# prannaykaul/lvc

Measured on AMD Instinct MI355X. Metric: img/s COCO 800x1333 R50-FPN inference (GeneralizedRCNN.forward(batched_inputs) -> Instances, 1000 proposals, 100 detections), higher is better.
Workload: dtype f32 (conv/GEMM inner products on the fp16 / bf16 matrix cores through fp32-accurate operand splits: two-way fp16 with main + cross fp32 accumulators for the 3x3 and wide 1x1 / FC layers, three-way bf16 for the rest; final boxes/scores closer to the fp64 evaluation than the reference's fp32 CPU path,; 1 GPU; COCO-detection R50-FPN inference, bs=8 synthetic 3x800x1333 per GPU, 1000 pre/post-NMS proposals per level/image, 80 classes, conditioned random-init weights; batch_per_gpu=8, global_batch=8, parallelism=dp1

## Files before the change

include/lvc_amd.h:

```cpp
#ifndef LVC_AMD_H
#define LVC_AMD_H

#ifdef __cplusplus
extern "C" {
#endif

#define LVC_OK 0
#define LVC_ERR_INVALID 1
#define LVC_ERR_HIP 2

int lvc_abi_version(void);
const char* lvc_last_error(void);
void lvc_set_error(const char* fmt, ...);

long long lvc_conv_workspace_bytes(void);
long long lvc_conv_range_words_offset(void);
void lvc_set_range_slot(int slot);
int lvc_range_slot(void);
int lvc_range_slots(void);
int lvc_conv2d_nhwc_f32(const float* x, const float* w_packed, const float* scale, const float* shift,
                        const float* residual, float* y, int N, int H, int W, int C, int K, int R, int S,
                        int stride, int pad, int Kg, int relu, int res_mode, int ldy, int ldr, int mode,
                        void* workspace, void* stream);

int lvc_conv2d_nhwc_bf16x3(const float* x, const unsigned short* w_split, const float* scale, const float* shift,
                           const float* residual, float* y, int N, int H, int W, int C, int K, int R, int S,
                           int stride, int pad, int Kg, int relu, int res_mode, int ldy, int ldr, void* workspace,
                           void* stream);

int lvc_conv3x3_nhwc_bf16x3(const float* x, const unsigned short* w_split, const float* scale, const float* shift,
                            const float* residual, float* y, int N, int H, int W, int C, int K, int Kg, int relu,
                            int res_mode, int ldy, int ldr, void* workspace, void* stream);

int lvc_conv3x3_nhwc_f16x2(const float* x, const unsigned short* w_split, const float* scale, const float* shift,
                           const float* residual, float* y, int N, int H, int W, int C, int K, int Kg, int relu,
                           int res_mode, int ldy, int ldr, void* workspace, void* stream);
int lvc_conv3x3_nhwc_f16s1(const float* x, const unsigned short* w_split, const float* scale, const float* shift,
                           const float* residual, float* y, int N, int H, int W, int C, int K, int Kg, int relu,
                           int res_mode, int ldy, int ldr, void* workspace, void* stream);
int lvc_conv3x3_nhwc_f16x2_pipe(const float* x, const unsigned short* w_split, const float* scale, const float* shift,
                                const float* residual, float* y, int N, int H, int W, int C, int K, int Kg, int relu,
                                int res_mode, int ldy, int ldr, void* workspace, void* stream);
int lvc_conv3x3_nhwc_f16_levels(int oneacc, const float* const* xs, float* const* ys, const int* Hs, const int* Ws, int L,
                                const unsigned short* w_split, const float* scale, const float* shift, int N, int C, int K, int Kg,
                                int relu, void* workspace, void* stream);
int lvc_conv3x3_nhwc_f16_levels_pred(int oneacc, const float* const* xs, float* const* ys, const int* Hs, const int* Ws, int L,
                                     const unsigned short* w_split, const float* scale, const float* shift, int N, int C, int K, int Kg,
                                     int relu, const unsigned short* pred_w, const float* pred_scale, const float* pred_shift, int pred_K,
                                     int pred_rows, int pred_ld, int pred_slot, void* workspace, void* stream);
int lvc_conv3x3_nhwc_f16_layers(int oneacc, const float* const* xs, float* const* ys, const int* Hs, const int* Ws, int L,
                                const unsigned short* const* ws, const float* const* scales, const float* const* shifts, int N, int C,
                                int K, int Kg, int relu, void* workspace, void* stream);
void lvc_set_wino_streamk(int mode);
void lvc_set_nms_reduce_global(int on);
void lvc_set_select_onelaunch(int mode);
int lvc_select_onelaunch(void);
void lvc_set_halo_test_hooks(int ph, int pw, int force);
int lvc_conv3x3_nhwc_wino(const float* x, const unsigned short* u, const float* scale, const float* shift, float* y, int N, int H, int W,
                          int C, int K, int Kpad, int relu, int ldy, void* workspace, void* stream);
int lvc_conv3x3_nhwc_wino_pred(const float* x, const unsigned short* u, const float* scale, const float* shift, float* y, int N, int H,
                               int W, int C, int K, int Kpad, int relu, int ldy, const unsigned short* pred_w, const float* pred_scale,
                               const float* pred_shift, int pred_K, int pred_rows, int pred_slot, void* workspace, void* stream);
int lvc_conv1x1_nhwc_f16x2_pipe(const float* x, const unsigned short* w_split, const float* scale, const float* shift,
                                const float* residual, float* y, int N, int H, int W, int C, int K, int stride, int relu,
                                int res_mode, int ldy, int ldr, void* workspace, void* stream);
int lvc_conv1x1_nhwc_f16s1(const float* x, const unsigned short* w_split, const float* scale, const float* shift,
                           const float* residual, float* y, int N, int H, int W, int C, int K, int stride, int relu,
                           int res_mode, int ldy, int ldr, void* workspace, void* stream);
int lvc_conv3x3_nhwc_f16s1_presplit(const float* x, const unsigned short* w_split, const float* scale, const float* shift, void* y,
                                    int N, int H, int W, int C, int K, int Kg, int next_slot, void* workspace, void* stream);
int lvc_conv1x1_nhwc_f16s1_presplit(const void* x, const unsigned short* w_split, const float* scale, const float* shift,
                                    const float* residual, float* y, int N, int H, int W, int C, int K, int relu,
                                    int res_mode, int ldy, int ldr, void* workspace, void* stream);
int lvc_conv1x1_nhwc_f16s1_w2(const float* x, const unsigned short* w_split, const float* scale, const float* shift,
                              const float* residual, float* y, int N, int H, int W, int C, int K, int Kpad, int stride, int relu,
                              int res_mode, int ldy, int ldr, void* workspace, void* stream);
int lvc_conv1x1_chain_nhwc_f16s1(const float* x, int ldx, const unsigned short* wa, int wa_rows, const float* sa, const float* ta,
                                 const float* residual, int ldr, float* y1, int ldy1, int relu1, const unsigned short* wb,
                                 int wb_rows, const float* sb, const float* tb, float* y2, int ldy2, int relu2, int M, int K1,
                                 int N1, int N2, void* workspace, void* stream);
int lvc_bottleneck_nhwc_f16s1(const float* x, int ldx, float* y, int ldy, int N, int H, int W, int cin, int proj,
                              const unsigned short* w, const float* s1, const float* t1, const float* s2, const float* t2,
                              const float* s3, const float* t3, void* workspace, void* stream);
int lvc_split_weights_rowscaled(const float* wp, int rows, int Kg, void* planes_out, float* row_factor, void* stream);

int lvc_conv2d_nhwc_f16x2(const float* x, const unsigned short* w_split, const float* scale, const float* shift,
                          const float* residual, float* y, int N, int H, int W, int C, int K, int R, int S,
                          int stride, int pad, int Kg, int relu, int res_mode, int ldy, int ldr, void* workspace,
                          void* stream);
int lvc_conv2d_nhwc_f16x2_dma(const float* x, const unsigned short* w_split, const float* scale, const float* shift,
                          const float* residual, float* y, int N, int H, int W, int C, int K, int R, int S,
                          int stride, int pad, int Kg, int relu, int res_mode, int ldy, int ldr, void* workspace,
                          void* stream);

int lvc_stem_conv_pool_nhwc4_f16x2(const float* x, const unsigned short* w_split, const float* scale, const float* shift,
                                   float* y, int N, int H, int W, int Kpad, int relu, int* d_error_word,
                                   float* y2 , int ldy2, void* stream);

int lvc_preprocess_nhwc4(const void* image, int dtype, int h, int w, const float* mean3, const float* std3,
                         float* out, int Hp, int Wp, void* stream);
int lvc_preprocess_batch_nhwc4(const void* const* images, int dtype, const int* hs, const int* ws, int B, const float* mean3,
                               const float* std3, float* out, int Hp, int Wp, void* stream);

int lvc_resize_bilinear_u8(const unsigned char* image, int H, int W, int new_h, int new_w, const int* xb, const int* xk,
                           int kxs, const int* yb, const int* yk, int kys, unsigned char* tmp, unsigned char* out_u8,
                           float* out_nhwc4, int Hp, int Wp, const float* mean3, const float* std3, void* stream);
int lvc_tta_resize_u8(const unsigned char* image, int H, int W, long long sy, long long sx, long long sc, const long long* hjobs,
                      int n_h, const long long* vjobs, int n_v, const float* mean3, const float* std3, void* stream);
long long lvc_tta_merge_workspace_bytes(int B, int Nmax);
int lvc_tta_merge(const float* boxes, const float* scores, const int* classes, const int* counts, int topk_in, const float* params,
                  const int* tab, int B, int Nmax, float score_thresh, double nms_thresh, int topk_out, float* ob, float* osc, int* ocl,
                  int* ocount, void* workspace, long long workspace_bytes, void* stream);
// ... 203 lines not shown
```

lvc_amd/_lib.py:

```python
import ctypes
import os

_HERE = os.path.dirname(os.path.abspath(__file__))
_SO = os.environ.get("LVC_AMD_LIB") or os.path.join(_HERE, "liblvc_amd.so")
_lib = None

c_void_p = ctypes.c_void_p
c_int = ctypes.c_int
c_float = ctypes.c_float
c_double = ctypes.c_double
c_longlong = ctypes.c_longlong


class LvcNativeError(RuntimeError):
    pass


def lib():
    global _lib
    if _lib is None:
        if not os.path.exists(_SO):
            raise ImportError(
                "lvc_amd: native library {} not found; build it with "
                "`python -c 'import __graft_entry__ as g; g.build()'` or `make -C lvc_amd/csrc` "
                "(there is no CPU fallback)".format(_SO)
            )
        L = ctypes.CDLL(_SO)
        L.lvc_last_error.restype = ctypes.c_char_p
        L.lvc_batched_nms_workspace_bytes.restype = c_longlong
        L.lvc_tta_merge_workspace_bytes.restype = c_longlong
        L.lvc_group_norm_workspace_bytes.restype = c_longlong
        L.lvc_abi_version.restype = c_int
        L.lvc_set_wino_streamk.restype = None
        if os.environ.get("LVC_WINO_STREAMK", "0") != "0":
            L.lvc_set_wino_streamk(c_int(int(os.environ["LVC_WINO_STREAMK"])))
        L.lvc_set_nms_reduce_global.restype = None
        L.lvc_set_halo_test_hooks.restype = None
        if os.environ.get("LVC_NMS_REDUCE_GLOBAL", "0") != "0":
            L.lvc_set_nms_reduce_global(c_int(1))
        L.lvc_set_select_onelaunch.restype = None
        if os.environ.get("LVC_SELECT_ONELAUNCH", "3") != "3":
            L.lvc_set_select_onelaunch(c_int(int(os.environ["LVC_SELECT_ONELAUNCH"])))
        _lib = L
    return _lib


def check(status, what=""):
    if status != 0:
        msg = lib().lvc_last_error().decode("utf-8", "replace")
        lib().lvc_set_range_slot(0)
        raise LvcNativeError("{} failed (status {}): {}".format(what or "lvc_amd native call", status, msg))


def ptr(t):
    if t is None:
        return c_void_p(0)
    return c_void_p(t.data_ptr())


def current_stream(device=None):
    import torch

    return c_void_p(torch.cuda.current_stream(device).cuda_stream)
```

lvc_amd/csrc/conv3x3_wino.hip:

```cpp
#include "conv_common.h"
#include <stdlib.h>
#include <type_traits>

#define WN_NT 512
#define WN_PAIRS 128
#define WN_CH 128
#define WN_VROWS 160
#define WN_PP (WN_VROWS * 32)
#define WN_VBUF (8 * WN_PP)
#define WN_USLOT (8 * WN_CH * 32)
#define WN_SMEM (2 * WN_VBUF + 2 * WN_USLOT)

struct WinoArgs {
  const float* x;
  const unsigned short* u;
  const float* scale;
  const float* shift;
  float* y;
  int* flags;
  float* partials;
  int N, H, W, C, K, Kpad, ldy, relu;
  int PH, PWP, lg_pwp, tiles_x, tiles_y, tiles_n, ntiles, nk, err_index;
  int units_per_worker, nworkers;
  unsigned x_bytes, y_bytes;
  const unsigned short* pred_w;
  const float* pred_scale;
  const float* pred_shift;
  long long pred_plane;
  int pred_K, pred_err_index;
};

template <bool PRED, bool SK>
__device__ __forceinline__ void wino_tile(const WinoArgs& p, const int t, const int cc0, const int cc1, const int lw, unsigned char* const smem) {
  unsigned char* const sV = smem;
  unsigned char* const sU = smem + 2 * WN_VBUF;

  int tid_ = threadIdx.x;
  if constexpr (SK) asm volatile("" : "+v"(tid_));
  const int tid = tid_;
  const int lane = tid & 63;
  const int wave = __builtin_amdgcn_readfirstlane(tid >> 6);
  const int ph = wave & 1, wn = (wave >> 1) & 1, wm = wave >> 2;
  const int fi = lane & 31, fh = lane >> 5;

  const int tn = t % p.tiles_n;
  int r0 = t / p.tiles_n;
  const int tx = r0 % p.tiles_x;
  r0 /= p.tiles_x;
  const int ty = r0 % p.tiles_y;
  const int img = r0 / p.tiles_y;
  const int y0 = ty * p.PH, x0 = tx * 2 * p.PWP, n0 = tn * WN_CH;
  const int VR = (p.PH + 2) * p.PWP;

  const __amdgpu_buffer_rsrc_t xres = __builtin_amdgcn_make_buffer_rsrc((void*)p.x, 0, p.x_bytes, 0x00020000);

  const int q = tid & 3;
  const unsigned pix_b = (unsigned)p.C * 4u;
  unsigned off0, mask0, off1[2];
  int lds0, lds1;
  bool on1;
  float sgn1;
  {
    const int vrow = tid >> 2;
    const int vy = vrow >> p.lg_pwp, vx = vrow & (p.PWP - 1);
    const int iy = y0 - 1 + vy, ix = x0 + 2 * vx - 1;
    unsigned m = 0;
#pragma unroll
    for (int j = 0; j < 4; ++j) m |= (iy >= 0 && iy < p.H && ix + j >= 0 && ix + j < p.W) ? (1u << j) : 0u;
    mask0 = m;
    off0 = (unsigned)((((long long)img * p.H + iy) * p.W + ix) * p.C + q * 4) * 4u;
    lds0 = vrow * 32 + (((q >> 1) ^ ((vrow >> 3) & 1)) << 4) + (q & 1) * 8;
  }
  {
    const int vrow = 128 + (tid >> 4), pz = (tid >> 2) & 3;
    on1 = vrow < VR;
    const int vy = vrow >> p.lg_pwp, vx = vrow & (p.PWP - 1);
    const int iy = y0 - 1 + vy, ix = x0 + 2 * vx - 1;
    const int ja = pz == 0 ? 0 : pz == 2 ? 2 : 1, jb = pz == 3 ? 3 : pz == 2 ? 1 : 2;
    sgn1 = pz == 1 ? 1.f : -1.f;
    const unsigned base = (unsigned)((((long long)img * p.H + iy) * p.W + ix) * p.C + q * 4) * 4u;
    const bool rowok = on1 && iy >= 0 && iy < p.H;
    off1[0] = (rowok && ix + ja >= 0 && ix + ja < p.W) ? base + (unsigned)ja * pix_b : 0x80000000u;
    off1[1] = (rowok && ix + jb >= 0 && ix + jb < p.W) ? base + (unsigned)jb * pix_b : 0x80000000u;
    lds1 = pz * WN_PP + vrow * 32 + (((q >> 1) ^ ((vrow >> 3) & 1)) << 4) + (q & 1) * 8;
  }
  f32x4 raw0[4], raw1[2];
  float big = 0.f;
  auto load0 = [&](int kc) {
#pragma unroll
    for (int j = 0; j < 4; ++j) {
      const unsigned off = ((mask0 >> j) & 1u) ? off0 + (unsigned)j * pix_b + (unsigned)kc * 64u : 0x80000000u;
      raw0[j] = __builtin_bit_cast(f32x4, __builtin_amdgcn_raw_buffer_load_b128(xres, off, 0, 0));
    }
  };
  auto load1 = [&](int kc) {
#pragma unroll
    for (int j = 0; j < 2; ++j) {
      const unsigned off = off1[j] == 0x80000000u ? 0x80000000u : off1[j] + (unsigned)kc * 64u;
      raw1[j] = __builtin_bit_cast(f32x4, __builtin_amdgcn_raw_buffer_load_b128(xres, off, 0, 0));
    }
  };
  f16x4 pk0[4][2], pk1[2];
  auto split = [&](f32x4 v, f16x4& h, f16x4& l) {
#pragma unroll
    for (int e = 0; e < 4; ++e) {
      const float a = v[e] * LVC_ACT_SCALE;
      const f16 hh = (f16)a;
      h[e] = hh;
      l[e] = (f16)(a - (float)hh);
      big = fmaxf(big, fabsf(v[e]));
    }
  };
  auto prep0 = [&]() {
    split(raw0[0] - raw0[2], pk0[0][0], pk0[0][1]);
    split(raw0[1] + raw0[2], pk0[1][0], pk0[1][1]);
    split(raw0[2] - raw0[1], pk0[2][0], pk0[2][1]);
    split(raw0[1] - raw0[3], pk0[3][0], pk0[3][1]);
  };
  auto write0 = [&](unsigned char* vb) {
#ifndef WN_DIAG_NO_LDSWRITE
#pragma unroll
    for (int pz = 0; pz < 4; ++pz) {
      *reinterpret_cast<f16x4*>(vb + pz * WN_PP + lds0) = pk0[pz][0];
      *reinterpret_cast<f16x4*>(vb + (4 + pz) * WN_PP + lds0) = pk0[pz][1];
    }
#endif
  };
  auto prep1 = [&]() { split(raw1[0] + sgn1 * raw1[1], pk1[0], pk1[1]); };
  auto write1 = [&](unsigned char* vb) {
#ifndef WN_DIAG_NO_LDSWRITE
    *reinterpret_cast<f16x4*>(vb + lds1) = pk1[0];
    *reinterpret_cast<f16x4*>(vb + 4 * WN_PP + lds1) = pk1[1];
#endif
  };
// ... 143 lines not shown
        for (int a = 0; a < 2; ++a)
#pragma unroll
          for (int b = 0; b < 2; ++b)
#pragma unroll
            for (int c = 0; c < 2; ++c) {
              f32x4 v[4];
#pragma unroll
              for (int e4 = 0; e4 < 4; ++e4)
                v[e4] = __builtin_bit_cast(f32x4, __builtin_amdgcn_raw_buffer_load_b128(pres, toff, ((((a * 2 + b) * 2 + c) * 4 + e4)) * WN_NT * 16, 0));
#pragma unroll
              for (int e4 = 0; e4 < 4; ++e4) {
                acc[a][b][c][e4 * 4 + 0] += v[e4][0]; acc[a][b][c][e4 * 4 + 1] += v[e4][1];
                acc[a][b][c][e4 * 4 + 2] += v[e4][2]; acc[a][b][c][e4 * 4 + 3] += v[e4][3];
              }
              __builtin_amdgcn_sched_barrier(0);
            }
        __syncthreads();
        if (tid == 0) lvc_release_partial(p.flags, pw);
      }
    }
  }

  float* xch = reinterpret_cast<float*>(smem);
  const int pair_slot = wm * 2 + wn;
  {
    float* mine = xch + ((size_t)(ph * 4 + pair_slot) * 4) * 1024;
    const int give = ph == 0 ? 1 : 0;
#pragma unroll
    for (int mi = 0; mi < 2; ++mi)
#pragma unroll
      for (int ni = 0; ni < 2; ++ni)
#pragma unroll
        for (int e = 0; e < 16; ++e) mine[((mi * 2 + ni) * 16 + e) * 64 + lane] = ph == 0 ? acc[1][mi][ni][e] : acc[0][mi][ni][e];
    (void)give;
  }
  __syncthreads();
  const float* theirs = xch + ((size_t)((1 - ph) * 4 + pair_slot) * 4) * 1024;
  const __amdgpu_buffer_rsrc_t yres = __builtin_amdgcn_make_buffer_rsrc((void*)p.y, 0, p.y_bytes, 0x00020000);
  float sc[2], sh[2];
#pragma unroll
  for (int ni = 0; ni < 2; ++ni) {
    const int ch = n0 + wn * 64 + ni * 32 + fi;
    sc[ni] = ch < p.K ? p.scale[ch] : 0.f;
    sh[ni] = (p.shift && ch < p.K) ? p.shift[ch] : 0.f;
  }
  if constexpr (!PRED) {
#pragma unroll
    for (int mi = 0; mi < 2; ++mi)
#pragma unroll
      for (int e = 0; e < 16; ++e) {
        const int m = wm * 64 + mi * 32 + (e & 3) + 8 * (e >> 2) + 4 * fh;
        const int py = m >> p.lg_pwp, px = m & (p.PWP - 1);
        const int oy = y0 + py, ox = x0 + 2 * px + ph;
        const bool ok = oy < p.H && ox < p.W;
#pragma unroll
        for (int ni = 0; ni < 2; ++ni) {
          const float o = theirs[((mi * 2 + ni) * 16 + e) * 64 + lane];
          float v = ph == 0 ? (acc[0][mi][ni][e] + acc[1][mi][ni][e]) + o : (o - acc[0][mi][ni][e]) - acc[1][mi][ni][e];
          v = v * sc[ni] + sh[ni];
          if (p.relu) v = v > 0.f ? v : 0.f;
          const int ch = n0 + wn * 64 + ni * 32 + fi;
          const unsigned off = (ok && ch < p.K) ? (unsigned)((((long long)img * p.H + oy) * p.W + ox) * p.ldy + ch) * 4u : 0xfffffff0u;
          __builtin_amdgcn_raw_buffer_store_b32(__builtin_bit_cast(unsigned, v), yres, off, 0, 0);
        }
      }
  } else {
    constexpr int CSS = WN_CH + 4;
    float bigp = 0.f;
#pragma unroll
    for (int mi = 0; mi < 2; ++mi)
#pragma unroll
      for (int e = 0; e < 16; ++e)
#pragma unroll
        for (int ni = 0; ni < 2; ++ni) {
          const float o = theirs[((mi * 2 + ni) * 16 + e) * 64 + lane];
          float v = ph == 0 ? (acc[0][mi][ni][e] + acc[1][mi][ni][e]) + o : (o - acc[0][mi][ni][e]) - acc[1][mi][ni][e];
          v = v * sc[ni] + sh[ni];
          if (p.relu) v = v > 0.f ? v : 0.f;
          bigp = (fabsf(v) > bigp || v != v) ? fabsf(v) : bigp;
          acc[0][mi][ni][e] = v;
        }
    __syncthreads();
    float* Cs = reinterpret_cast<float*>(smem);
#pragma unroll
    for (int mi = 0; mi < 2; ++mi)
#pragma unroll
      for (int e = 0; e < 16; ++e) {
        const int m = wm * 64 + mi * 32 + (e & 3) + 8 * (e >> 2) + 4 * fh;
#pragma unroll
        for (int ni = 0; ni < 2; ++ni) Cs[(2 * m + ph) * CSS + wn * 64 + ni * 32 + fi] = acc[0][mi][ni][e];
      }
    __syncthreads();
    const unsigned short* bsrcp = p.pred_w + (size_t)fi * p.K + n0 + fh * 8;
    f16x8 pbh = *reinterpret_cast<const f16x8*>(bsrcp), pbl = *reinterpret_cast<const f16x8*>(bsrcp + p.pred_plane);
    f32x16 pm, px2;
#pragma unroll
    for (int e = 0; e < 16; ++e) { pm[e] = 0.f; px2[e] = 0.f; }
    const float* arow = Cs + (wave * 32 + fi) * CSS + fh * 8;
#pragma unroll 1
    for (int ks = 0; ks < WN_CH / 16; ++ks) {
      const int kn = ks + 1 < WN_CH / 16 ? ks + 1 : ks;
      const f16x8 nbh = *reinterpret_cast<const f16x8*>(bsrcp + kn * 16);
      const f16x8 nbl = *reinterpret_cast<const f16x8*>(bsrcp + p.pred_plane + kn * 16);
      const f32x4 a0 = *reinterpret_cast<const f32x4*>(arow + ks * 16);
      const f32x4 a1 = *reinterpret_cast<const f32x4*>(arow + ks * 16 + 4);
      f16x8 ah, al;
#pragma unroll
      for (int j = 0; j < 8; ++j) {
        const float a = j < 4 ? a0[j & 3] : a1[j & 3];
        const f16 hh = (f16)a;
        ah[j] = hh;
        al[j] = (f16)((a - (float)hh) * 2048.f);
      }
      pm = __builtin_amdgcn_mfma_f32_32x32x16_f16(ah, pbh, pm, 0, 0, 0);
      px2 = __builtin_amdgcn_mfma_f32_32x32x16_f16(al, pbh, px2, 0, 0, 0);
      px2 = __builtin_amdgcn_mfma_f32_32x32x16_f16(ah, pbl, px2, 0, 0, 0);
      pbh = nbh; pbl = nbl;
    }
    float* rblk = Cs + wave * 32 * CSS;
#pragma unroll
    for (int e = 0; e < 16; ++e) rblk[((e & 3) + 8 * (e >> 2) + 4 * fh) * 32 + fi] = pm[e] + px2[e] * (1.f / 2048.f);
    __builtin_amdgcn_fence(__ATOMIC_RELEASE, "workgroup");
    __builtin_amdgcn_wave_barrier();
    if (fi < p.pred_K) {
      const float psc = p.pred_scale ? p.pred_scale[fi] : 1.f;
      const float psh = (n0 == 0 && p.pred_shift) ? p.pred_shift[fi] : 0.f;
#pragma unroll 2
      for (int rr = 0; rr < 32; rr += 2) {
        const int r = wave * 32 + rr + fh;
        const int m = r >> 1;
        const int oy = y0 + (m >> p.lg_pwp), ox = x0 + 2 * (m & (p.PWP - 1)) + (r & 1);
        const float v = rblk[(rr + fh) * 32 + fi];
        if (oy < p.H && ox < p.W) unsafeAtomicAdd(p.y + ((size_t)((long long)img * p.H + oy) * p.W + ox) * p.ldy + fi, v * psc + psh);
      }
    }
    lvc_report_range(p.flags, p.pred_err_index, bigp, LVC_F16_MAX);
  }
}

template <bool PRED>
__global__ __launch_bounds__(WN_NT, 2) void conv3x3_wino_kernel(WinoArgs p) {
  __shared__ __attribute__((aligned(1024))) unsigned char smem[WN_SMEM];
  wino_tile<PRED, false>(p, lvc_xcd_remap(blockIdx.x, p.ntiles), 0, p.nk, 0, smem);
}

template <bool PRED, bool SPLIT>
__global__ __launch_bounds__(WN_NT, 2) void conv3x3_wino_sk_kernel(WinoArgs p) {
  __shared__ __attribute__((aligned(1024))) unsigned char smem[WN_SMEM];
  const int lw = lvc_xcd_remap(blockIdx.x, p.nworkers);
  int u = lw * p.units_per_worker;
  const int u_end = min(u + p.units_per_worker, p.ntiles * p.nk);
#pragma unroll 1
  while (u < u_end) {
    const int t = u / p.nk, cc0 = u - t * p.nk;
    const int cc1 = min(p.nk, cc0 + (u_end - u));
    if constexpr (SPLIT) wino_tile<PRED, true>(p, t, cc0, cc1, lw, smem);
    else wino_tile<PRED, false>(p, t, 0, p.nk, lw, smem);
    __syncthreads();
    u += cc1 - cc0;
  }
}

static int g_wino_streamk = 0;
extern "C" void lvc_set_wino_streamk(int mode) { g_wino_streamk = mode; }

static int wn_cus() {
  const int cus = lvc_cu_count() / 8 * 8;
  return cus < 8 ? 8 : cus;
}

static int wino_launch(const float* x, const unsigned short* u, const float* scale, const float* shift, float* y, int N, int H, int W, int C,
                       int K, int Kpad, int relu, int ldy, const unsigned short* pred_w, const float* pred_scale, const float* pred_shift,
                       int pred_K, int pred_rows, int pred_slot, void* workspace, void* stream) {
  LVC_CHECK_ARG(x && u && scale && y && workspace, "null pointer");
  LVC_CHECK_ARG(N > 0 && H > 0 && W > 0 && C > 0 && K > 0, "non-positive dimension");
  LVC_CHECK_ARG(C % 16 == 0 && Kpad % WN_CH == 0 && Kpad >= K, "needs C % 16 == 0 and weight planes padded to 128 rows");
  WinoArgs a;
  a.x = x; a.u = u; a.scale = scale; a.shift = shift; a.y = y;
  a.N = N; a.H = H; a.W = W; a.C = C; a.K = K; a.Kpad = Kpad; a.ldy = ldy > 0 ? ldy : K; a.relu = relu;
  const long long xb = (long long)N * H * W * C * 4, yb = (long long)N * H * W * a.ldy * 4;
  LVC_CHECK_ARG(xb < (1ll << 31) && yb < (1ll << 31), "tensors must be smaller than 2 GiB");
  a.x_bytes = (unsigned)xb; a.y_bytes = (unsigned)yb;
  auto waste = [&](int phh, int pwp) { return (long long)lvc_cdiv(H, phh) * phh * lvc_cdiv(W, 2 * pwp) * 2 * pwp; };
  if (waste(16, 8) < waste(8, 16)) { a.PH = 16; a.PWP = 8; a.lg_pwp = 3; } else { a.PH = 8; a.PWP = 16; a.lg_pwp = 4; }
  a.tiles_x = lvc_cdiv(W, 2 * a.PWP); a.tiles_y = lvc_cdiv(H, a.PH); a.tiles_n = lvc_cdiv(K, WN_CH);
  const long long nt = (long long)N * a.tiles_x * a.tiles_y * a.tiles_n;
  LVC_CHECK_ARG(nt < (1ll << 31), "too many tiles");
  a.ntiles = (int)nt;
  a.nk = C / 16;
  a.flags = lvc_ws_flags(workspace);
  a.err_index = lvc_ws_range_index(lvc_range_slot());
  a.pred_w = pred_w; a.pred_scale = pred_scale; a.pred_shift = pred_shift; a.pred_K = pred_K;
  a.pred_plane = (long long)pred_rows * K;
  a.pred_err_index = lvc_ws_range_index(pred_slot);
  if (pred_w) {
    LVC_CHECK_ARG(K % WN_CH == 0 && K <= 2 * WN_CH, "the pointwise layer on top needs 128 or 256 hidden channels (at most two slices per output)");
    LVC_CHECK_ARG(pred_K >= 1 && pred_K <= 32 && pred_rows >= 32 && pred_slot >= 0 && pred_slot < lvc_range_slots(), "bad pointwise layer");
  }
  a.partials = (float*)workspace;
  const long long nunits = (long long)a.ntiles * a.nk;
  const int cus = wn_cus() < LVC_MAX_WORKERS / 2 ? wn_cus() : LVC_MAX_WORKERS / 2;
  bool sk = g_wino_streamk != 0 && nunits < (1ll << 31) && a.ntiles % cus != 0;
  if (sk) {
    constexpr int min_units = 4;
    lvc_plan_workers(nunits, cus, min_units, &a.units_per_worker, &a.nworkers);
    const bool whole = g_wino_streamk == 2;
    if (whole) {
      a.units_per_worker = (a.units_per_worker + a.nk - 1) / a.nk * a.nk;
      a.nworkers = (int)((nunits + a.units_per_worker - 1) / a.units_per_worker);
    }
    if (pred_w) {
      if (whole) hipLaunchKernelGGL((conv3x3_wino_sk_kernel<true, false>), dim3(a.nworkers), dim3(WN_NT), 0, (hipStream_t)stream, a);
      else hipLaunchKernelGGL((conv3x3_wino_sk_kernel<true, true>), dim3(a.nworkers), dim3(WN_NT), 0, (hipStream_t)stream, a);
    } else {
      if (whole) hipLaunchKernelGGL((conv3x3_wino_sk_kernel<false, false>), dim3(a.nworkers), dim3(WN_NT), 0, (hipStream_t)stream, a);
      else hipLaunchKernelGGL((conv3x3_wino_sk_kernel<false, true>), dim3(a.nworkers), dim3(WN_NT), 0, (hipStream_t)stream, a);
    }
  } else {
    a.units_per_worker = a.nk; a.nworkers = a.ntiles;
    if (pred_w) hipLaunchKernelGGL(conv3x3_wino_kernel<true>, dim3(a.ntiles), dim3(WN_NT), 0, (hipStream_t)stream, a);
    else hipLaunchKernelGGL(conv3x3_wino_kernel<false>, dim3(a.ntiles), dim3(WN_NT), 0, (hipStream_t)stream, a);
  }
  LVC_CHECK_LAUNCH();
  return LVC_OK;
}

extern "C" int lvc_conv3x3_nhwc_wino(const float* x, const unsigned short* u, const float* scale, const float* shift, float* y, int N, int H,
                                     int W, int C, int K, int Kpad, int relu, int ldy, void* workspace, void* stream) {
  return wino_launch(x, u, scale, shift, y, N, H, W, C, K, Kpad, relu, ldy, nullptr, nullptr, nullptr, 0, 0, 0, workspace, stream);
}

extern "C" int lvc_conv3x3_nhwc_wino_pred(const float* x, const unsigned short* u, const float* scale, const float* shift, float* y, int N,
                                          int H, int W, int C, int K, int Kpad, int relu, int ldy, const unsigned short* pred_w,
                                          const float* pred_scale, const float* pred_shift, int pred_K, int pred_rows, int pred_slot,
                                          void* workspace, void* stream) {
  LVC_CHECK_ARG(pred_w, "null pointer");
  return wino_launch(x, u, scale, shift, y, N, H, W, C, K, Kpad, relu, ldy, pred_w, pred_scale, pred_shift, pred_K, pred_rows, pred_slot, workspace,
                     stream);
}
```

lvc_amd/kernels.py:

```python
import collections
import ctypes

import torch

from . import _lib
from ._lib import LvcNativeError, c_double, c_float, c_int, c_longlong, c_void_p, check, ptr

BK = 32
BN = 128


def _stream(t):
    return c_void_p(torch.cuda.current_stream(t.device).cuda_stream)


def _req_cuda(*ts):
    for t in ts:
        if t is not None and not t.is_cuda:
            raise RuntimeError("lvc_amd kernels need device tensors (got a CPU tensor); there is no CPU path")


class PackedConv:

    __slots__ = ("w", "scale", "shift", "K", "C", "R", "S", "stride", "pad", "Kg", "mode", "_w3", "_w2h", "_w2s", "two_acc",
# ... 645 lines not shown
            code, act = 2, None
        operand, tail, last = _CONV_ARGS[entry]

        def call():
            wts, scale = (pc.split2s() if operand == "s" else
                          ((pc.split2h() if operand == "h" else pc.split3() if operand == "3" else pc.w), pc.scale))
            ints = (N, H, W, C, pc.K) + tail(pc, wts) + (code, res_mode, ldo, ldr) + last(pc)
            return getattr(_lib.lib(), entry)(ptr(x), ptr(wts), ptr(scale), ptr(pc.shift), ptr(residual), ptr(out),
                                              *[c_int(v) for v in ints], ptr(conv_workspace(x.device)), _stream(x))
    c_real = 3 if pc.mode == 1 else C
    nbytes = 4.0 * (N * (Ho * Wo if (pc.R == 1 and pc.S == 1) else H * W) * c_real + N * Ho * Wo * pc.K + res_numel
                    + pc.K * c_real * pc.R * pc.S)
    if grouped:
        c_real = C // pc.groups
        nbytes = 4.0 * (N * H * W * C + N * Ho * Wo * pc.K + res_numel + pc.K * c_real * 9)
    _launch(route.engine, 2.0 * N * Ho * Wo * pc.K * c_real * pc.R * pc.S, nbytes, pc.slot if route.slotted else None, entry, call)
    if act == "gelu":
        check(_lib.lib().lvc_gelu(ptr(out), ptr(out), c_longlong(out.numel()), _stream(out)), "lvc_gelu")
    elif act is not None:
        raise ValueError("unknown activation {!r}".format(act))
    return out


class PackedChain:

    __slots__ = ("wa", "sa", "ta", "wb", "sb", "tb", "K1", "N1", "N2", "slot", "state", "__weakref__")


_PERM16 = (0, 1, 2, 3, 8, 9, 10, 11, 4, 5, 6, 7, 12, 13, 14, 15)
CHAIN_SHAPES = {(64, 256, 64), (128, 256, 64), (128, 512, 128)}


def _chain_planes(pc):
    assert pc.R == 1 and pc.S == 1 and pc.mode == 0 and pc.stride == 1 and pc.pad == 0
    rows, Kg = pc.w.shape
    idx = torch.arange(Kg, device=pc.w.device).view(-1, 16)[:, list(_PERM16)].reshape(-1)
    wperm = pc.w[:, idx].contiguous()
    planes = torch.empty((2, rows, Kg), device=pc.w.device, dtype=torch.float16)
    fac = torch.empty(rows, device=pc.w.device, dtype=torch.float32)
    check(_lib.lib().lvc_split_weights_rowscaled(ptr(wperm), c_int(rows), c_int(Kg), ptr(planes), ptr(fac), _stream(pc.w)),
          "lvc_split_weights_rowscaled")
    fac = fac[: pc.K]
    return planes, (fac * pc.scale if pc.scale is not None else fac).contiguous()


CONV_WINO = _os.environ.get("LVC_CONV_WINO", "1") != "0"
WINO_STREAMK = int(_os.environ.get("LVC_WINO_STREAMK", "0"))


def set_wino_streamk(mode):
    global WINO_STREAMK
    WINO_STREAMK = int(mode)
    _lib.lib().lvc_set_wino_streamk(c_int(int(mode)))
WINO_RPN = False
_WINO_MIN_TILES = 512


def pack_wino(pc):
    cached = pc.state.get("_wino")
    if cached is not None and cached[0] is pc.w:
        return cached[1], cached[2]
    assert pc.R == 3 and pc.S == 3 and pc.mode == 0 and pc.C % 32 == 0
    K, C = pc.K, pc.C
    w = pc.w[:K].view(K, C // 32, 3, 3, 32).permute(0, 1, 4, 2, 3).reshape(K, C, 3, 3).double()
    g0, g1, g2 = w[..., 0], w[..., 1], w[..., 2]
    U = torch.stack([g0, (g0 + g1 + g2) / 2, (g0 - g1 + g2) / 2, g2], dim=-1).float()
    Kpad = (K + 127) // 128 * 128
    flat = torch.zeros(Kpad, C * 12, device=pc.w.device)
    flat[:K] = U.reshape(K, C * 12)
    planes = torch.empty(2, Kpad, C * 12, dtype=torch.int16, device=pc.w.device)
    fac = torch.empty(Kpad, device=pc.w.device)
    check(_lib.lib().lvc_split_weights_rowscaled(ptr(flat), c_int(Kpad), c_int(C * 12), ptr(planes), ptr(fac), _stream(flat)), "lvc_split_weights_rowscaled")
    u = planes.view(2, Kpad, C // 16, 16, 3, 4).permute(4, 2, 5, 0, 1, 3).contiguous()
    scale = (fac[:K] * pc.scale if pc.scale is not None else fac[:K]).contiguous()
    pc.state["_wino"] = (pc.w, u, scale)
    return u, scale


def _wino_launch(x, pc, relu, out):
    _req_cuda(x)
    N, H, W, C = x.shape
    u, scale = pack_wino(pc)
    return _lib.lib().lvc_conv3x3_nhwc_wino(ptr(x), ptr(u), ptr(scale), ptr(pc.shift), ptr(out), c_int(N), c_int(H), c_int(W), c_int(C), c_int(pc.K),
                                            c_int(u.shape[4]), c_int(1 if relu else 0), c_int(out.stride(2)), ptr(conv_workspace(x.device)), _stream(x))


def conv3x3_wino(x, pc, relu=False, out=None):
    if out is None:
        out = torch.empty(x.shape[0], x.shape[1], x.shape[2], pc.K, device=x.device, dtype=torch.float32)
    check(_wino_launch(x, pc, relu, out), "lvc_conv3x3_nhwc_wino")
    return out


def wino_tiles(N, H, W, K):
    return N * ((H + 7) // 8) * ((W + 31) // 32) * ((K + 127) // 128)


def _direct_f16_3x3(pc, C):
    return (CONV_ENGINE == "bf16x3" and CONV_SPLIT == "f16x2" and CONV_HALO and HALO_S1 >= 1 and pc.state["tier"] < 2 and pc.mode == 0
            and pc.R == 3 and pc.S == 3 and pc.stride == 1 and pc.pad == 1 and pc.C == C and C % 32 == 0)


def _level_maps_ok(xs, N, C, K):
    return (all(x.dim() == 4 and x.is_contiguous() and x.dtype == torch.float32 and x.shape[0] == N and x.shape[3] == C
                and x.numel() < (1 << 29) for x in xs)
            and halo_tiles(N, max(x.shape[1] * x.shape[2] for x in xs), K) >= _HALO_H2_MIN_TILES)


def _wino_levels(xs, K):
    big = [i for i, x in enumerate(xs) if wino_sized(x.shape[0], x.shape[1], x.shape[2], K)]
    return big, [i for i in range(len(xs)) if i not in big]


_GROUP_SLOTS = {}


def _group_slot(pcs):
    key = tuple(id(pc.state) for pc in pcs)
    ent = _GROUP_SLOTS.get(key)
    if ent is None or any(r() is None for r in ent[1]):
        import weakref

        slot = _new_range_slot(pcs[0])
        for pc in pcs[1:]:
            _SLOT_OWNERS[slot].append(weakref.ref(pc))
        if len(_GROUP_SLOTS) > 64:
            _GROUP_SLOTS.clear()
        ent = _GROUP_SLOTS[key] = (slot, [weakref.ref(pc) for pc in pcs])
    else:
        import weakref

        live = [r for r in _SLOT_OWNERS.get(ent[0], []) if r() is not None and all(r() is not pc for pc in pcs)]
        _SLOT_OWNERS[ent[0]] = live + [weakref.ref(pc) for pc in pcs]
    return ent[0]


def conv3x3_levels(xs, pc, relu=False, outs=None):
    _req_cuda(*xs)
    pcs = list(pc) if isinstance(pc, (list, tuple)) else [pc] * len(xs)
    shared = not isinstance(pc, (list, tuple))
    p0 = pcs[0]
    N, C = xs[0].shape[0], xs[0].shape[3]
    if outs is None:
        outs = [torch.empty(x.shape[0], x.shape[1], x.shape[2], q.K, device=x.device, dtype=torch.float32) for x, q in zip(xs, pcs)]
    forms = {(q.two_acc or q.state["tier"] >= 1) for q in pcs}
    ok = (len(xs) > 1 and len(xs) <= 6 and len(pcs) == len(xs) and len(forms) == 1
          and all(_direct_f16_3x3(q, C) and q.K == p0.K and q.Kg == p0.Kg for q in pcs) and p0.K >= 64 and p0.K % 4 == 0
          and _level_maps_ok(xs, N, C, p0.K)
          and all(o.is_contiguous() and o.shape == (x.shape[0], x.shape[1], x.shape[2], p0.K) for o, x in zip(outs, xs)))
    if not ok:
        for x, q, o in zip(xs, pcs, outs):
            conv2d_nhwc(x, q, relu=relu, out=o)
        return outs
    one = HALO_S1 == 2 and not (True in forms)
    if CONV_WINO and HALO_S1 == 2 and all(q.state["tier"] == 0 and (not q.two_acc or WINO_RPN) for q in pcs):
        big, rest = _wino_levels(xs, p0.K)
        if big:
            for i in big:
                conv2d_nhwc(xs[i], pcs[i], relu=relu, out=outs[i])
            if rest:
                conv3x3_levels([xs[i] for i in rest], pc if shared else [pcs[i] for i in rest], relu=relu, outs=[outs[i] for i in rest])
            return outs
    L = len(xs)
    XP, IP = c_void_p * L, c_int * L
    xp, yp = XP(*[x.data_ptr() for x in xs]), XP(*[o.data_ptr() for o in outs])
    hs, ws = IP(*[x.shape[1] for x in xs]), IP(*[x.shape[2] for x in xs])
    for q in pcs:
        q.last_one = one
    ops = [q.split2s() if one else (q.split2h(), q.scale) for q in (pcs[:1] if shared else pcs)]
    if shared:
        weights = (ptr(ops[0][0]), ptr(ops[0][1]), ptr(p0.shift))
    else:
        weights = [XP(*[0 if t is None else t.data_ptr() for t in ts]) for ts in ([o[0] for o in ops], [o[1] for o in ops], [q.shift for q in pcs])]
    entry = "lvc_conv3x3_nhwc_f16_levels" if shared else "lvc_conv3x3_nhwc_f16_layers"
    px = sum(x.shape[0] * x.shape[1] * x.shape[2] for x in xs)
    _launch("f16x2_halo", 2.0 * px * p0.K * C * 9, 4.0 * (px * C + px * p0.K + (1 if shared else L) * p0.K * C * 9),
            p0.slot if shared else _group_slot(pcs), entry, lambda: getattr(_lib.lib(), entry)(
                c_int(1 if one else 0), xp, yp, hs, ws, c_int(L), *weights, c_int(N), c_int(C), c_int(p0.K), c_int(p0.Kg),
                c_int(1 if relu else 0), ptr(conv_workspace(xs[0].device)), _stream(xs[0])))
    return outs


def conv3x3_levels_pred(xs, pc, pred, relu=True, _outs=None):
    _req_cuda(*xs)
    N, C = xs[0].shape[0], xs[0].shape[3]
    ok = (1 <= len(xs) <= 6 and _direct_f16_3x3(pc, C)
          and (pc.two_acc or pc.state["tier"] == 1 or HALO_S1 == 1)
          and pc.K in (128, 256) and pc.Kg == 9 * C
          and pred.mode == 0 and pred.R == 1 and pred.S == 1 and pred.stride == 1 and pred.pad == 0 and pred.C == pc.K and pred.Kg == pc.K
          and 1 <= pred.K <= 32 and pred.w.shape[0] >= 32 and pred.state["tier"] < 2
          and _level_maps_ok(xs, N, C, pc.K))
    if not ok:
        return None
    ms = [x.shape[0] * x.shape[1] * x.shape[2] for x in xs]
    if _outs is None:
        y = torch.zeros(sum(ms), pred.K, device=xs[0].device, dtype=torch.float32)
        outs, off = [], 0
        for x, m in zip(xs, ms):
            outs.append(y[off:off + m].view(x.shape[0], x.shape[1], x.shape[2], pred.K))
            off += m
    else:
        outs = _outs
    if CONV_WINO and WINO_RPN and HALO_S1 == 2 and pc.state["tier"] == 0:
        big, rest = _wino_levels(xs, pc.K)
        if big:
            u, scale = pack_wino(pc)
            pplanes = pred.split2h()
            pc.last_one = True
            pred.last_one = False
            for i in big:
                x, o = xs[i], outs[i]
                px = x.shape[0] * x.shape[1] * x.shape[2]
# ... 1971 lines not shown
```

Baseline: 662.4 img/s.

## Group multi-level Winograd 3x3 convs into one stacked-row launch

```diff
diff --git a/include/lvc_amd.h b/include/lvc_amd.h
--- a/include/lvc_amd.h
+++ b/include/lvc_amd.h
@@ -58,6 +58,10 @@
 void lvc_set_halo_test_hooks(int ph, int pw, int force);
 int lvc_conv3x3_nhwc_wino(const float* x, const unsigned short* u, const float* scale, const float* shift, float* y, int N, int H, int W,
                           int C, int K, int Kpad, int relu, int ldy, void* workspace, void* stream);
+int lvc_conv3x3_nhwc_wino_layers(const float* const* xs, float* const* ys, const int* Hs, const int* Ws, int L,
+                                 const unsigned short* const* us, const float* const* scales, const float* const* shifts, int N, int C,
+                                 int K, int Kpad, int relu, void* workspace, void* stream);
+void lvc_set_wino_group(int mode);
 int lvc_conv3x3_nhwc_wino_pred(const float* x, const unsigned short* u, const float* scale, const float* shift, float* y, int N, int H,
                                int W, int C, int K, int Kpad, int relu, int ldy, const unsigned short* pred_w, const float* pred_scale,
                                const float* pred_shift, int pred_K, int pred_rows, int pred_slot, void* workspace, void* stream);
diff --git a/lvc_amd/_lib.py b/lvc_amd/_lib.py
--- a/lvc_amd/_lib.py
+++ b/lvc_amd/_lib.py
@@ -34,6 +34,9 @@
         L.lvc_set_wino_streamk.restype = None
         if os.environ.get("LVC_WINO_STREAMK", "0") != "0":
             L.lvc_set_wino_streamk(c_int(int(os.environ["LVC_WINO_STREAMK"])))
+        L.lvc_set_wino_group.restype = None
+        if os.environ.get("LVC_WINO_GROUP", "1") != "1":
+            L.lvc_set_wino_group(c_int(int(os.environ["LVC_WINO_GROUP"])))
         L.lvc_set_nms_reduce_global.restype = None
         L.lvc_set_halo_test_hooks.restype = None
         if os.environ.get("LVC_NMS_REDUCE_GLOBAL", "0") != "0":
diff --git a/lvc_amd/csrc/conv3x3_wino.hip b/lvc_amd/csrc/conv3x3_wino.hip
--- a/lvc_amd/csrc/conv3x3_wino.hip
+++ b/lvc_amd/csrc/conv3x3_wino.hip
@@ -1,5 +1,6 @@
 #include "conv_common.h"
 #include <stdlib.h>
+#include <string.h>
 #include <type_traits>
 
 #define WN_NT 512
@@ -28,9 +29,29 @@
   const float* pred_shift;
   long long pred_plane;
   int pred_K, pred_err_index;
+  int vrows, hp1;
+  unsigned magic;
 };
 
-template <bool PRED, bool SK>
+struct WinoMap {
+  const float* x;
+  const unsigned short* u;
+  const float* scale;
+  const float* shift;
+  float* y;
+  int H, W, ldy, PH, PWP, lg_pwp, tiles_x, tile0, vrows, hp1;
+  unsigned magic, x_bytes, y_bytes;
+};
+
+#define WN_MAX_MAPS 4
+struct WinoGroupArgs {
+  WinoMap m[WN_MAX_MAPS];
+  int tile_end[WN_MAX_MAPS - 1];
+  int* flags;
+  int N, C, K, Kpad, relu, tiles_n, ntiles, nk, err_index;
+};
+
+template <bool PRED, bool SK, bool STACK = false>
 __device__ __forceinline__ void wino_tile(const WinoArgs& p, const int t, const int cc0, const int cc1, const int lw, unsigned char* const smem) {
   unsigned char* const sV = smem;
   unsigned char* const sU = smem + 2 * WN_VBUF;
@@ -47,8 +68,13 @@
   int r0 = t / p.tiles_n;
   const int tx = r0 % p.tiles_x;
   r0 /= p.tiles_x;
-  const int ty = r0 % p.tiles_y;
-  const int img = r0 / p.tiles_y;
+  const int ty = STACK ? r0 : r0 % p.tiles_y;
+  const int img = STACK ? 0 : r0 / p.tiles_y;
+  static_assert(!(STACK && (PRED || SK)), "stacked rows: the plain epilogue on whole tiles only");
+  auto srow = [&](int v) {
+    const int im = (int)__umulhi((unsigned)v, p.magic);
+    return (v >= 0 && v < p.vrows && v - im * p.hp1 < p.H) ? v - im : -1;
+  };
   const int y0 = ty * p.PH, x0 = tx * 2 * p.PWP, n0 = tn * WN_CH;
   const int VR = (p.PH + 2) * p.PWP;
 
@@ -64,11 +90,13 @@
     const int vrow = tid >> 2;
     const int vy = vrow >> p.lg_pwp, vx = vrow & (p.PWP - 1);
     const int iy = y0 - 1 + vy, ix = x0 + 2 * vx - 1;
+    const long long gy = STACK ? (long long)srow(iy) : (long long)img * p.H + iy;
+    const bool rowok = STACK ? gy >= 0 : (iy >= 0 && iy < p.H);
     unsigned m = 0;
 #pragma unroll
-    for (int j = 0; j < 4; ++j) m |= (iy >= 0 && iy < p.H && ix + j >= 0 && ix + j < p.W) ? (1u << j) : 0u;
+    for (int j = 0; j < 4; ++j) m |= (rowok && ix + j >= 0 && ix + j < p.W) ? (1u << j) : 0u;
     mask0 = m;
-    off0 = (unsigned)((((long long)img * p.H + iy) * p.W + ix) * p.C + q * 4) * 4u;
+    off0 = (unsigned)((gy * p.W + ix) * p.C + q * 4) * 4u;
     lds0 = vrow * 32 + (((q >> 1) ^ ((vrow >> 3) & 1)) << 4) + (q & 1) * 8;
   }
   {
@@ -78,8 +106,9 @@
     const int iy = y0 - 1 + vy, ix = x0 + 2 * vx - 1;
     const int ja = pz == 0 ? 0 : pz == 2 ? 2 : 1, jb = pz == 3 ? 3 : pz == 2 ? 1 : 2;
     sgn1 = pz == 1 ? 1.f : -1.f;
-    const unsigned base = (unsigned)((((long long)img * p.H + iy) * p.W + ix) * p.C + q * 4) * 4u;
-    const bool rowok = on1 && iy >= 0 && iy < p.H;
+    const long long gy = STACK ? (long long)srow(iy) : (long long)img * p.H + iy;
+    const unsigned base = (unsigned)((gy * p.W + ix) * p.C + q * 4) * 4u;
+    const bool rowok = on1 && (STACK ? gy >= 0 : (iy >= 0 && iy < p.H));
     off1[0] = (rowok && ix + ja >= 0 && ix + ja < p.W) ? base + (unsigned)ja * pix_b : 0x80000000u;
     off1[1] = (rowok && ix + jb >= 0 && ix + jb < p.W) ? base + (unsigned)jb * pix_b : 0x80000000u;
     lds1 = pz * WN_PP + vrow * 32 + (((q >> 1) ^ ((vrow >> 3) & 1)) << 4) + (q & 1) * 8;
@@ -329,7 +358,8 @@
         const int m = wm * 64 + mi * 32 + (e & 3) + 8 * (e >> 2) + 4 * fh;
         const int py = m >> p.lg_pwp, px = m & (p.PWP - 1);
         const int oy = y0 + py, ox = x0 + 2 * px + ph;
-        const bool ok = oy < p.H && ox < p.W;
+        const long long gy = STACK ? (long long)srow(y0 + ((wm * 64 + mi * 32 + 8 * (e >> 2)) >> p.lg_pwp)) : (long long)img * p.H + oy;
+        const bool ok = (STACK ? gy >= 0 : oy < p.H) && ox < p.W;
 #pragma unroll
         for (int ni = 0; ni < 2; ++ni) {
           const float o = theirs[((mi * 2 + ni) * 16 + e) * 64 + lane];
@@ -337,7 +367,7 @@
           v = v * sc[ni] + sh[ni];
           if (p.relu) v = v > 0.f ? v : 0.f;
           const int ch = n0 + wn * 64 + ni * 32 + fi;
-          const unsigned off = (ok && ch < p.K) ? (unsigned)((((long long)img * p.H + oy) * p.W + ox) * p.ldy + ch) * 4u : 0xfffffff0u;
+          const unsigned off = (ok && ch < p.K) ? (unsigned)((gy * p.W + ox) * p.ldy + ch) * 4u : 0xfffffff0u;
           __builtin_amdgcn_raw_buffer_store_b32(__builtin_bit_cast(unsigned, v), yres, off, 0, 0);
         }
       }
@@ -421,6 +451,25 @@
   wino_tile<PRED, false>(p, lvc_xcd_remap(blockIdx.x, p.ntiles), 0, p.nk, 0, smem);
 }
 
+__global__ __launch_bounds__(WN_NT, 2) void conv3x3_wino_group_kernel(WinoGroupArgs g) {
+  __shared__ __attribute__((aligned(1024))) unsigned char smem[WN_SMEM];
+  const int t = lvc_xcd_remap(blockIdx.x, g.ntiles);
+  WinoMap m = g.m[0];
+#pragma unroll
+  for (int i = 1; i < WN_MAX_MAPS; ++i)
+    if (t >= g.tile_end[i - 1]) m = g.m[i];
+  WinoArgs p;
+  p.x = m.x; p.u = m.u; p.scale = m.scale; p.shift = m.shift; p.y = m.y;
+  p.flags = g.flags; p.partials = nullptr;
+  p.N = g.N; p.H = m.H; p.W = m.W; p.C = g.C; p.K = g.K; p.Kpad = g.Kpad; p.ldy = m.ldy; p.relu = g.relu;
+  p.PH = m.PH; p.PWP = m.PWP; p.lg_pwp = m.lg_pwp; p.tiles_x = m.tiles_x; p.tiles_y = 0; p.tiles_n = g.tiles_n; p.ntiles = g.ntiles;
+  p.nk = g.nk; p.err_index = g.err_index; p.units_per_worker = g.nk; p.nworkers = g.ntiles;
+  p.x_bytes = m.x_bytes; p.y_bytes = m.y_bytes;
+  p.pred_w = nullptr; p.pred_scale = nullptr; p.pred_shift = nullptr; p.pred_plane = 0; p.pred_K = 0; p.pred_err_index = 0;
+  p.vrows = m.vrows; p.hp1 = m.hp1; p.magic = m.magic;
+  wino_tile<false, false, true>(p, t - m.tile0, 0, g.nk, 0, smem);
+}
+
 template <bool PRED, bool SPLIT>
 __global__ __launch_bounds__(WN_NT, 2) void conv3x3_wino_sk_kernel(WinoArgs p) {
   __shared__ __attribute__((aligned(1024))) unsigned char smem[WN_SMEM];
@@ -440,10 +489,57 @@
 
 static int g_wino_streamk = 0;
 extern "C" void lvc_set_wino_streamk(int mode) { g_wino_streamk = mode; }
+static int g_wino_group = 1;
+extern "C" void lvc_set_wino_group(int mode) { g_wino_group = mode; }
 
 static int wn_cus() {
   const int cus = lvc_cu_count() / 8 * 8;
   return cus < 8 ? 8 : cus;
+}
+
+static bool wino_stack_ok(int N, int H) { return ((long long)N * (H + 1) + 32) * (H + 1) < (1ll << 32); }
+
+static int wino_group_launch(const float* const* xs, float* const* ys, const int* Hs, const int* Ws, const int* ldys, int L,
+                             const unsigned short* const* us, const float* const* scales, const float* const* shifts, int N, int C, int K,
+                             int Kpad, int relu, void* workspace, void* stream) {
+  WinoGroupArgs g;
+  memset(&g, 0, sizeof(g));
+  g.N = N; g.C = C; g.K = K; g.Kpad = Kpad; g.relu = relu; g.nk = C / 16; g.tiles_n = lvc_cdiv(K, WN_CH);
+  g.flags = lvc_ws_flags(workspace);
+  g.err_index = lvc_ws_range_index(lvc_range_slot());
+  long long tiles[WN_MAX_MAPS];
+  for (int l = 0; l < L; ++l) {
+    WinoMap& m = g.m[l];
+    const int H = Hs[l], W = Ws[l];
+    LVC_CHECK_ARG(H > 0 && W > 0, "non-positive dimension");
+    LVC_CHECK_ARG(ldys[l] >= K, "output rows narrower than K");
+    m.x = xs[l]; m.u = us[l]; m.scale = scales[l]; m.shift = shifts ? shifts[l] : nullptr; m.y = ys[l];
+    m.H = H; m.W = W; m.ldy = ldys[l];
+    const long long xb = (long long)N * H * W * C * 4, yb = (long long)N * H * W * m.ldy * 4;
+    LVC_CHECK_ARG(xb < (1ll << 31) && yb < (1ll << 31), "tensors must be smaller than 2 GiB");
+    LVC_CHECK_ARG(wino_stack_ok(N, H), "map too tall for stacked rows");
+    m.x_bytes = (unsigned)xb; m.y_bytes = (unsigned)yb;
+    m.hp1 = H + 1; m.vrows = N * (H + 1) - 1; m.magic = (unsigned)((1ull << 32) / (unsigned)(H + 1) + 1);
+    auto waste = [&](int phh, int pwp) { return (long long)lvc_cdiv(m.vrows, phh) * phh * lvc_cdiv(W, 2 * pwp) * 2 * pwp; };
+    if (waste(16, 8) < waste(8, 16)) { m.PH = 16; m.PWP = 8; m.lg_pwp = 3; } else { m.PH = 8; m.PWP = 16; m.lg_pwp = 4; }
+    m.tiles_x = lvc_cdiv(W, 2 * m.PWP);
+    tiles[l] = (long long)lvc_cdiv(m.vrows, m.PH) * m.tiles_x * g.tiles_n;
+  }
+  for (int l = 1; l < L; ++l)
+    for (int j = l; j > 0 && tiles[j] > tiles[j - 1]; --j) {
+      const WinoMap tm = g.m[j]; g.m[j] = g.m[j - 1]; g.m[j - 1] = tm;
+      const long long tt = tiles[j]; tiles[j] = tiles[j - 1]; tiles[j - 1] = tt;
+    }
+  long long nt = 0;
+  for (int l = 0; l < WN_MAX_MAPS; ++l) {
+    if (l < L) { g.m[l].tile0 = (int)nt; nt += tiles[l]; LVC_CHECK_ARG(nt < (1ll << 31), "too many tiles"); }
+    else g.m[l] = g.m[0];
+    if (l < WN_MAX_MAPS - 1) g.tile_end[l] = l < L - 1 ? (int)nt : 0x7fffffff;
+  }
+  g.ntiles = (int)nt;
+  hipLaunchKernelGGL(conv3x3_wino_group_kernel, dim3(g.ntiles), dim3(WN_NT), 0, (hipStream_t)stream, g);
+  LVC_CHECK_LAUNCH();
+  return LVC_OK;
 }
 
 static int wino_launch(const float* x, const unsigned short* u, const float* scale, const float* shift, float* y, int N, int H, int W, int C,
@@ -452,6 +548,10 @@
   LVC_CHECK_ARG(x && u && scale && y && workspace, "null pointer");
   LVC_CHECK_ARG(N > 0 && H > 0 && W > 0 && C > 0 && K > 0, "non-positive dimension");
   LVC_CHECK_ARG(C % 16 == 0 && Kpad % WN_CH == 0 && Kpad >= K, "needs C % 16 == 0 and weight planes padded to 128 rows");
+  if (!pred_w && g_wino_group != 0 && g_wino_streamk == 0 && wino_stack_ok(N, H)) {
+    const int ld = ldy > 0 ? ldy : K;
+    return wino_group_launch(&x, &y, &H, &W, &ld, 1, &u, &scale, &shift, N, C, K, Kpad, relu, workspace, stream);
+  }
   WinoArgs a;
   a.x = x; a.u = u; a.scale = scale; a.shift = shift; a.y = y;
   a.N = N; a.H = H; a.W = W; a.C = C; a.K = K; a.Kpad = Kpad; a.ldy = ldy > 0 ? ldy : K; a.relu = relu;
@@ -507,6 +607,30 @@
   return wino_launch(x, u, scale, shift, y, N, H, W, C, K, Kpad, relu, ldy, nullptr, nullptr, nullptr, 0, 0, 0, workspace, stream);
 }
 
+extern "C" int lvc_conv3x3_nhwc_wino_layers(const float* const* xs, float* const* ys, const int* Hs, const int* Ws, int L,
+                                            const unsigned short* const* us, const float* const* scales, const float* const* shifts, int N,
+                                            int C, int K, int Kpad, int relu, void* workspace, void* stream) {
+  LVC_CHECK_ARG(xs && ys && Hs && Ws && us && scales && workspace, "null pointer");
+  LVC_CHECK_ARG(L >= 1 && L <= WN_MAX_MAPS, "1 to 4 maps");
+  LVC_CHECK_ARG(N > 0 && C > 0 && K > 0, "non-positive dimension");
+  LVC_CHECK_ARG(C % 16 == 0 && Kpad % WN_CH == 0 && Kpad >= K, "needs C % 16 == 0 and weight planes padded to 128 rows");
+  bool group = g_wino_group != 0 && g_wino_streamk == 0;
+  int ldys[WN_MAX_MAPS];
+  for (int l = 0; l < L; ++l) {
+    LVC_CHECK_ARG(xs[l] && ys[l] && us[l] && scales[l], "null pointer");
+    LVC_CHECK_ARG(Hs[l] > 0 && Ws[l] > 0, "non-positive dimension");
+    group = group && wino_stack_ok(N, Hs[l]);
+    ldys[l] = K;
+  }
+  if (group) return wino_group_launch(xs, ys, Hs, Ws, ldys, L, us, scales, shifts, N, C, K, Kpad, relu, workspace, stream);
+  for (int l = 0; l < L; ++l) {
+    const int st = wino_launch(xs[l], us[l], scales[l], shifts ? shifts[l] : nullptr, ys[l], N, Hs[l], Ws[l], C, K, Kpad, relu, K, nullptr, nullptr,
+                               nullptr, 0, 0, 0, workspace, stream);
+    if (st != LVC_OK) return st;
+  }
+  return LVC_OK;
+}
+
 extern "C" int lvc_conv3x3_nhwc_wino_pred(const float* x, const unsigned short* u, const float* scale, const float* shift, float* y, int N,
                                           int H, int W, int C, int K, int Kpad, int relu, int ldy, const unsigned short* pred_w,
                                           const float* pred_scale, const float* pred_shift, int pred_K, int pred_rows, int pred_slot,
diff --git a/lvc_amd/kernels.py b/lvc_amd/kernels.py
--- a/lvc_amd/kernels.py
+++ b/lvc_amd/kernels.py
@@ -721,6 +721,18 @@
     global WINO_STREAMK
     WINO_STREAMK = int(mode)
     _lib.lib().lvc_set_wino_streamk(c_int(int(mode)))
+
+
+WINO_GROUP = int(_os.environ.get("LVC_WINO_GROUP", "1"))
+_WINO_GROUP_MAX = 4
+
+
+def set_wino_group(mode):
+    global WINO_GROUP
+    WINO_GROUP = int(mode)
+    _lib.lib().lvc_set_wino_group(c_int(int(mode)))
+
+
 WINO_RPN = False
 _WINO_MIN_TILES = 512
 
@@ -802,6 +814,24 @@
         live = [r for r in _SLOT_OWNERS.get(ent[0], []) if r() is not None and all(r() is not pc for pc in pcs)]
         _SLOT_OWNERS[ent[0]] = live + [weakref.ref(pc) for pc in pcs]
     return ent[0]
+
+
+def _wino_layers_launch(xs, pcs, shared, relu, outs):
+    L = len(xs)
+    N, C = xs[0].shape[0], xs[0].shape[3]
+    p0 = pcs[0]
+    ops = [pack_wino(q) for q in (pcs[:1] * L if shared else pcs)]
+    XP, IP = c_void_p * L, c_int * L
+    xp, yp = XP(*[x.data_ptr() for x in xs]), XP(*[o.data_ptr() for o in outs])
+    hs, ws = IP(*[x.shape[1] for x in xs]), IP(*[x.shape[2] for x in xs])
+    up, sp, tp = (XP(*[0 if t is None else t.data_ptr() for t in ts]) for ts in ([o[0] for o in ops], [o[1] for o in ops], [q.shift for q in pcs]))
+    for q in pcs:
+        q.last_one = True
+    px = sum(x.shape[0] * x.shape[1] * x.shape[2] for x in xs)
+    _launch("f16x2_wino", 2.0 * px * p0.K * C * 9, 4.0 * (px * C + px * p0.K + (1 if shared else L) * p0.K * C * 9),
+            p0.slot if shared else _group_slot(pcs), "lvc_conv3x3_nhwc_wino_layers", lambda: _lib.lib().lvc_conv3x3_nhwc_wino_layers(
+                xp, yp, hs, ws, c_int(L), up, sp, tp, c_int(N), c_int(C), c_int(p0.K), c_int(ops[0][0].shape[4]), c_int(1 if relu else 0),
+                ptr(conv_workspace(xs[0].device)), _stream(xs[0])))
 
 
 def conv3x3_levels(xs, pc, relu=False, outs=None):
@@ -825,8 +855,11 @@
     if CONV_WINO and HALO_S1 == 2 and all(q.state["tier"] == 0 and (not q.two_acc or WINO_RPN) for q in pcs):
         big, rest = _wino_levels(xs, p0.K)
         if big:
-            for i in big:
-                conv2d_nhwc(xs[i], pcs[i], relu=relu, out=outs[i])
+            if WINO_GROUP and not WINO_STREAMK and 1 < len(big) <= _WINO_GROUP_MAX:
+                _wino_layers_launch([xs[i] for i in big], [pcs[i] for i in big], shared, relu, [outs[i] for i in big])
+            else:
+                for i in big:
+                    conv2d_nhwc(xs[i], pcs[i], relu=relu, out=outs[i])
             if rest:
                 conv3x3_levels([xs[i] for i in rest], pc if shared else [pcs[i] for i in rest], relu=relu, outs=[outs[i] for i in rest])
             return outs
```

Result: no change. 665.1 img/s (median of 2 runs) (+0.4%).
